# stevewongv/Sparse2Dense

Measured on AMD Instinct MI355X. Metric: LiDAR frames/sec (fwd+bwd), 150k-pt 0.1m-voxel synthetic Waymo scene, higher is better.
Workload: dtype bf16 (sparse stack: bf16 storage; dense neck/head: bf16 NHWC activations; fp32 accumulate, statistics, master weights, optimizer)

## Files before the change

include/s2d.h:

```cpp
#ifndef S2D_H_
#define S2D_H_

#include <stddef.h>
#include <stdint.h>

#ifdef __cplusplus
extern "C" {
#endif

typedef void *s2d_stream_t;

#define S2D_OK 0
#define S2D_ERR_INVALID_ARG (-1)
#define S2D_ERR_UNSUPPORTED (-2)
#define S2D_ERR_CAPACITY (-3)
#define S2D_ERR_WORKSPACE (-4)
#define S2D_ERR_COMM (-5)

int s2d_version(void);
int s2d_last_error(char *buf, size_t buf_len);
int s2d_build_info(char *buf, size_t buf_len);

size_t s2d_voxelize_batch_workspace_bytes(int frames, const int64_t *point_offsets, int max_points, int max_voxels);
int s2d_voxelize_batch_run(const float *points, int frames, const int64_t *point_offsets, int ndim,
// ... 179 lines not shown
                             s2d_stream_t stream);
int s2d_bnrow_apply_ld_bf16(const void *x, const float *scale, const float *shift, const void *residual, int relu, int64_t n, int c, void *y,
                            int y_ld, s2d_stream_t stream);
int s2d_bnrow_bwd_reduce_ld_bf16(const void *dy, int dy_ld, const void *x, const void *y, const float *scale, const float *shift, int relu,
                                 int64_t n, int c, float *sums, float *sums_copy, void *ws, size_t ws_bytes, s2d_stream_t stream);
int s2d_bnrow_bwd_reduce_finalize_ld_bf16(const void *dy, int dy_ld, const void *x, const void *y, const float *scale, const float *shift,
                                          int relu, int64_t n, int c, const float *gamma, const float *mean, const float *invstd,
                                          float *dgamma, float *dbeta, float *a, float *b, float *d, void *ws, size_t ws_bytes,
                                          s2d_stream_t stream);
int s2d_bnrow_bwd_apply_ld_bf16(const void *dy, int dy_ld, const void *x, const void *y, const float *scale, const float *shift, int relu,
                                const float *a, const float *b, const float *d, int64_t n, int c, void *dx, void *dres,
                                s2d_stream_t stream);

int s2d_spconv_s16_supported(int cin, int cout);
size_t s2d_spconv_s16_packed_elems(int kvol, int cin, int cout);
int s2d_spconv_s16_pack_weights(const float *weight, int kvol, int cin, int cout, int transpose,
                                int flip, int64_t n_out, void *packed, s2d_stream_t stream);
int s2d_spconv_s16_pack_weights_pair(const float *weight, int kvol, int cin, int cout, int flip_dgrad, int64_t n_out_fwd, int64_t n_out_dgrad,
                                     void *packed_fwd, void *packed_dgrad, s2d_stream_t stream);
int s2d_spconv_s16_wgrad(const void *in_feat, int64_t n_in, const void *dout, const int32_t *nbr,
                         int64_t n_out, int kvol, int cin, int cout, float *dweight, void *ws,
                         size_t ws_bytes, s2d_stream_t stream);
int s2d_spconv_s16_fwd(const void *in_feat, int64_t n_in, const void *packed_weight,
                       const float *bias, const int32_t *nbr, int64_t n_out, int kvol, int cin,
                       int cout, const void *zero_page, void *out_feat, s2d_stream_t stream);
int64_t s2d_spconv_s16_stats_tiles(int64_t n_out, int kvol, int cin, int cout);
int s2d_spconv_s16_fwd_stats(const void *in_feat, int64_t n_in, const void *packed_weight, const float *bias, const int32_t *nbr,
                             int64_t n_out, int kvol, int cin, int cout, const void *zero_page, void *out_feat, float *stats_partial,
                             s2d_stream_t stream);

int s2d_spconv_s16_set_sorted_rows(int on);
size_t s2d_rulebook_sort_workspace_bytes(int64_t n);
int64_t s2d_rulebook_sort_chunk_rows(int64_t n);
int s2d_rulebook_sort_by_mask(const int32_t *nbr, int kvol, int64_t n, int32_t *perm, uint32_t *pmask, int32_t *nbr_perm, void *ws,
                              size_t ws_bytes, s2d_stream_t stream);
int s2d_spconv_s16_sorted_supported(int kvol, int cin, int cout);
int s2d_spconv_s16_fwd_sorted(const void *in_feat, int64_t n_in, const void *packed_weight, const float *bias, const int32_t *nbr_perm,
                              const int32_t *perm, const uint32_t *pmask, int64_t n_out, int kvol, int cin, int cout, void *out_feat,
                              float *stats_partial, s2d_stream_t stream);

int s2d_conv2d3x3_wgrad_supported(int cin, int cout);
size_t s2d_conv2d3x3_wgrad_workspace_bytes(int n_img, int h, int w, int cin, int cout, int pad);
int s2d_conv2d3x3_wgrad_nhwc_bf16(const void *x, const void *dy, const void *zero_page, int n_img,
                                  int h, int w, int cin, int cout, int pad, float *dweight, float *dbias , void *ws,
                                  size_t ws_bytes, s2d_stream_t stream);

int s2d_conv2d1x1_pack_weights_bf16(const float *weight, int cin, int cout, int transpose, void *packed, s2d_stream_t stream);
int s2d_conv2d3x3_pack_weights_pair_bf16(const float *weight, int cin, int cout, int weight_nhwc, void *packed_fwd, void *packed_dgrad,
                                         s2d_stream_t stream);
int s2d_conv2d1x1_pack_weights_pair_bf16(const float *weight, int cin, int cout, void *packed_fwd, void *packed_dgrad, s2d_stream_t stream);
int64_t s2d_conv2d1x1_stats_tiles(int n_img, int h, int w, int cin, int cout);
int s2d_conv2d1x1_nhwc_bf16(const void *x, const void *packed_weight, const float *bias, const void *zero_page, int n_img,
                            int h, int w, int cin, int cout, void *y, float *stats_partial, s2d_stream_t stream);
size_t s2d_conv2d1x1_wgrad_workspace_bytes(int n_img, int h, int w, int cin, int cout);
int s2d_conv2d1x1_wgrad_nhwc_bf16(const void *x, const void *dy, const void *zero_page, int n_img, int h, int w, int cin,
                                  int cout, float *dweight, float *dbias , void *ws, size_t ws_bytes, s2d_stream_t stream);

int s2d_smallconv3x3_supported(int cin, int cout);
int s2d_smallconv3x3_fwd(const void *x, const float *weight, const float *bias, int n_img, int h, int w, int cin, int cout, float *y,
                         s2d_stream_t stream);
int s2d_smallconv3x3_dgrad(const float *dy, const float *weight, int n_img, int h, int w, int cin, int cout, void *dx,
                           s2d_stream_t stream);
size_t s2d_smallconv3x3_wgrad_workspace_bytes(int cin, int cout);
int s2d_smallconv3x3_wgrad(const void *x, const float *dy, int n_img, int h, int w, int cin, int cout, float *dweight, float *dbias,
                           void *ws, size_t ws_bytes, s2d_stream_t stream);

int s2d_conv2d2x2s2_pack_weights_bf16(const float *weight, int cin, int cout, int weight_nhwc, void *packed, s2d_stream_t stream);
int64_t s2d_conv2d2x2s2_stats_tiles(int n_img, int h, int w);
int s2d_conv2d2x2s2_nhwc_bf16(const void *x, const void *packed_weight, const float *bias, const void *zero_page, int n_img,
                              int h, int w, int cin, int cout, void *y, float *stats_partial, s2d_stream_t stream);

int s2d_convup_supported(int kc, int nc, int ks);
int s2d_convup_pack_weights_bf16(const float *weight, int kc, int nc, int ks, void *packed, s2d_stream_t stream);
int64_t s2d_convup_stats_tiles(int n_img, int h, int w, int kc, int nc, int ks);
int s2d_convup_nhwc_bf16(const void *x, const void *packed_weight, const float *bias, const void *zero_page, int n_img, int h, int w,
                         int kc, int nc, int ks, void *y, float *stats_partial, s2d_stream_t stream);
int s2d_conv2d4x4s2_pack_weights_bf16(const float *weight, int cin, int cout, void *packed, s2d_stream_t stream);
int s2d_conv2d4x4s2_nhwc_bf16(const void *x, const void *packed_weight, const void *zero_page, int n_img, int h, int w, int cin,
                              int cout, void *y, s2d_stream_t stream);
int s2d_conv2d_s2_wgrad_supported(int ca, int cb, int ks);
size_t s2d_conv2d_s2_wgrad_workspace_bytes(int n_img, int h, int w, int ca, int cb, int ks);
int s2d_conv2d_s2_wgrad_nhwc_bf16(const void *a, const void *b, const void *zero_page, int n_img, int h, int w, int ca, int cb, int ks,
                                  float *dweight, void *ws, size_t ws_bytes, s2d_stream_t stream);

int s2d_rows_wgrad_supported(int ci, int co);
size_t s2d_rows_wgrad_workspace_bytes(int64_t rows, int ci, int co);
int s2d_rows_wgrad_f32(const float *x, const float *dy, int64_t rows, int ci, int co, float *dweight, void *ws, size_t ws_bytes,
                       s2d_stream_t stream);

int s2d_dwconv7_supported(int channels);
int s2d_dwconv7_nhwc_bf16(const void *x, const float *weight, const float *bias, int n_img, int h, int w,
                          int c, int flip, void *y, s2d_stream_t stream);
size_t s2d_dwconv7_wgrad_workspace_bytes(int n_img, int h, int w, int c);
int s2d_dwconv7_wgrad_nhwc_bf16(const void *x, const void *dy, int n_img, int h, int w, int c,
                                float *dweight, float *dbias, void *ws, size_t ws_bytes,
                                s2d_stream_t stream);

int s2d_convt3d_mfma_supported(int cin, int cout);
size_t s2d_convt3d_mfma_packed_elems(int cin, int cout);
int s2d_convt3d_mfma_pack_weights(const float *weight, int cin, int cout, void *packed, s2d_stream_t stream);
int s2d_convt3d_mfma_fwd(const float *in, const void *packed, const float *bias, int batch, int cin, int cout,
                         int d, int h, int w, float *out, s2d_stream_t stream);
int64_t s2d_convt3d_mfma_stats_tiles(int batch, int cin, int d, int h, int w);
int s2d_convt3d_mfma_fwd_stats(const float *in, const void *packed, const float *bias, int batch, int cin, int cout,
                               int d, int h, int w, float *out, float *stats_partial, s2d_stream_t stream);
int s2d_convt3d_mfma_dgrad(const float *dout, const void *packed, int batch, int cin, int cout, int d, int h,
// ... 398 lines not shown
```

sparse2dense_amd/_lib.py:

```python
import ctypes
import os

_HERE = os.path.dirname(os.path.abspath(__file__))
LIB_PATH = os.path.join(_HERE, "lib", "libs2d_hip.so")

c_i32p = ctypes.c_void_p
c_f32p = ctypes.c_void_p
_I3 = ctypes.c_int32 * 3
_PFN_GEO = [ctypes.c_int64, ctypes.c_int, ctypes.c_int, ctypes.c_float, ctypes.c_float, ctypes.c_float, ctypes.c_float]
_F3 = ctypes.c_float * 3
_F6 = ctypes.c_float * 6


class CenterTask(ctypes.Structure):
    _fields_ = [(n, ctypes.c_void_p) for n in ("hm_logit", "reg", "height", "dim", "vel", "rot", "hm", "ind", "mask", "cat", "anno_box", "p",
                                               "d_logit", "d_reg", "d_height", "d_dim", "d_vel", "d_rot")] + [("classes", ctypes.c_int)]

class CenterPredictTask(ctypes.Structure):
    _fields_ = [("map", ctypes.c_void_p * 6), ("channel_stride", ctypes.c_int64 * 6), ("pixel_stride", ctypes.c_int64 * 6),
                ("classes", ctypes.c_int), ("label_base", ctypes.c_int)]


class AnchorPredictTask(ctypes.Structure):
    _fields_ = [(n, ctypes.c_void_p) for n in ("box_preds", "cls_preds", "dir_cls_preds", "anchors")] + \
# ... 94 lines not shown
                                              ctypes.c_int64, c_f32p, ctypes.c_void_p]),
    "s2d_comm_load_library": (ctypes.c_int, [ctypes.c_char_p]),
    "s2d_comm_available": (ctypes.c_int, []),
    "s2d_comm_unique_id": (ctypes.c_int, [ctypes.c_void_p]),
    "s2d_comm_init": (ctypes.c_int, [ctypes.c_void_p, ctypes.c_int, ctypes.c_int]),
    "s2d_comm_ranks": (ctypes.c_int, []),
    "s2d_comm_shutdown": (ctypes.c_int, []),
    "s2d_convt3d_mfma_supported": (ctypes.c_int, [ctypes.c_int, ctypes.c_int]),
    "s2d_convt3d_mfma_packed_elems": (ctypes.c_size_t, [ctypes.c_int, ctypes.c_int]),
    "s2d_convt3d_mfma_pack_weights": (ctypes.c_int, [c_f32p, ctypes.c_int, ctypes.c_int, ctypes.c_void_p, ctypes.c_void_p]),
    "s2d_convt3d_mfma_fwd": (ctypes.c_int, [c_f32p, ctypes.c_void_p, c_f32p] + [ctypes.c_int] * 6 + [c_f32p, ctypes.c_void_p]),
    "s2d_convt3d_mfma_stats_tiles": (ctypes.c_int64, [ctypes.c_int] * 5),
    "s2d_convt3d_mfma_fwd_stats": (ctypes.c_int, [c_f32p, ctypes.c_void_p, c_f32p] + [ctypes.c_int] * 6 + [c_f32p, c_f32p, ctypes.c_void_p]),
    "s2d_convt3d_mfma_fwd_stats_y16": (ctypes.c_int, [c_f32p, ctypes.c_void_p, c_f32p] + [ctypes.c_int] * 6 + [c_f32p, c_f32p, ctypes.c_void_p]),
    "s2d_convt3d_mfma_d16_supported": (ctypes.c_int, [ctypes.c_int] * 5),
    "s2d_convt3d_mfma_dgrad_d16": (ctypes.c_int, [ctypes.c_void_p, ctypes.c_void_p] + [ctypes.c_int] * 6 + [c_f32p, ctypes.c_void_p]),
    "s2d_convt3d_mfma_wgrad_d16": (ctypes.c_int, [c_f32p, ctypes.c_void_p] + [ctypes.c_int] * 6 + [c_f32p, ctypes.c_void_p, ctypes.c_size_t,
                                                                                                   ctypes.c_void_p]),
    "s2d_convt3d_mfma_norm_supported": (ctypes.c_int, [ctypes.c_int] * 5),
    "s2d_convt3d_mfma_fwd_stats_y16_norm": (ctypes.c_int, [c_f32p, c_f32p, ctypes.c_void_p, c_f32p] + [ctypes.c_int] * 6 + [ctypes.c_void_p, c_f32p,
                                                                                                                  ctypes.c_void_p]),
    "s2d_convt3d_mfma_wgrad_d16_norm": (ctypes.c_int, [c_f32p, c_f32p, ctypes.c_void_p] + [ctypes.c_int] * 6 + [c_f32p, ctypes.c_void_p, ctypes.c_size_t,
                                                                                                              ctypes.c_void_p]),
    "s2d_convt3d_mfma_dgrad": (ctypes.c_int, [c_f32p, ctypes.c_void_p] + [ctypes.c_int] * 6 + [c_f32p, ctypes.c_void_p]),
    "s2d_convt3d_mfma_wgrad_workspace_bytes": (ctypes.c_size_t, [ctypes.c_int] * 6),
    "s2d_convt3d_mfma_wgrad": (ctypes.c_int, [c_f32p, c_f32p] + [ctypes.c_int] * 6 + [c_f32p, ctypes.c_void_p, ctypes.c_size_t,
                                                                                     ctypes.c_void_p]),
    "s2d_pointwise_conv_wgrad_workspace_bytes": (ctypes.c_size_t, [ctypes.c_int, ctypes.c_int]),
    "s2d_pointwise_conv_wgrad_f32": (ctypes.c_int, [c_f32p, c_f32p, ctypes.c_int, ctypes.c_int, ctypes.c_int, ctypes.c_int64, c_f32p, c_f32p,
                                                    ctypes.c_void_p, ctypes.c_size_t, ctypes.c_void_p]),
    "s2d_pointwise_conv_wgrad_bf16_supported": (ctypes.c_int, [ctypes.c_int, ctypes.c_int, ctypes.c_int64]),
    "s2d_pointwise_conv_wgrad_norm_bf16": (ctypes.c_int, [c_f32p, c_f32p, c_f32p, ctypes.c_int, ctypes.c_int, ctypes.c_int, ctypes.c_int64, c_f32p,
                                                          c_f32p, ctypes.c_void_p, ctypes.c_size_t, ctypes.c_void_p]),
    "s2d_pointwise_conv_wgrad_norm_x16": (ctypes.c_int, [c_f32p, c_f32p, c_f32p, ctypes.c_int, ctypes.c_int, ctypes.c_int, ctypes.c_int64, c_f32p,
                                                          c_f32p, ctypes.c_void_p, ctypes.c_size_t, ctypes.c_void_p]),
    "s2d_pointwise_conv_wgrad_bf16": (ctypes.c_int, [c_f32p, c_f32p, ctypes.c_int, ctypes.c_int, ctypes.c_int, ctypes.c_int64, c_f32p, c_f32p,
                                                     ctypes.c_void_p, ctypes.c_size_t, ctypes.c_void_p]),
    "s2d_pcr_loss_workspace_bytes": (ctypes.c_size_t, []),
    "s2d_pcr_loss_fwd_f32": (ctypes.c_int, [c_f32p, c_f32p, c_i32p, c_f32p, ctypes.c_int64] + [ctypes.c_int] * 4 +
                             [c_f32p, ctypes.c_void_p, ctypes.c_size_t, ctypes.c_void_p]),
    "s2d_pcr_loss_bwd_f32": (ctypes.c_int, [c_f32p, c_f32p, c_i32p, c_f32p, ctypes.c_int64] + [ctypes.c_int] * 4 +
                             [c_f32p, c_f32p, c_f32p, c_f32p, c_f32p, ctypes.c_void_p]),
    "s2d_nhwc_bf16_to_nchw_f32": (ctypes.c_int, [ctypes.c_void_p, ctypes.c_int, ctypes.c_int, ctypes.c_int64, c_f32p, ctypes.c_void_p]),
    "s2d_nchw_f32_to_nhwc_bf16": (ctypes.c_int, [c_f32p, ctypes.c_int, ctypes.c_int, ctypes.c_int64, ctypes.c_void_p, ctypes.c_void_p]),
    "s2d_nhwc_bf16_to_nchw_f32_ld": (ctypes.c_int, [ctypes.c_void_p, ctypes.c_int, ctypes.c_int, ctypes.c_int, ctypes.c_int64, c_f32p, ctypes.c_void_p]),
    "s2d_nchw_f32_to_nhwc_bf16_ld": (ctypes.c_int, [c_f32p, ctypes.c_int, ctypes.c_int, ctypes.c_int, ctypes.c_int64, ctypes.c_void_p, ctypes.c_void_p]),
    "s2d_conv2d1x1_pack_weights_bf16": (ctypes.c_int, [c_f32p, ctypes.c_int, ctypes.c_int, ctypes.c_int, ctypes.c_void_p, ctypes.c_void_p]),
    "s2d_conv2d3x3_pack_weights_pair_bf16": (ctypes.c_int, [c_f32p, ctypes.c_int, ctypes.c_int, ctypes.c_int, ctypes.c_void_p, ctypes.c_void_p,
                                                            ctypes.c_void_p]),
    "s2d_conv2d1x1_pack_weights_pair_bf16": (ctypes.c_int, [c_f32p, ctypes.c_int, ctypes.c_int, ctypes.c_void_p, ctypes.c_void_p, ctypes.c_void_p]),
    "s2d_conv2d1x1_stats_tiles": (ctypes.c_int64, [ctypes.c_int] * 5),
    "s2d_conv2d1x1_nhwc_bf16": (ctypes.c_int, [ctypes.c_void_p, ctypes.c_void_p, c_f32p, ctypes.c_void_p] + [ctypes.c_int] * 5 +
                                [ctypes.c_void_p, c_f32p, ctypes.c_void_p]),
    "s2d_conv2d1x1_wgrad_workspace_bytes": (ctypes.c_size_t, [ctypes.c_int] * 5),
    "s2d_conv2d1x1_wgrad_nhwc_bf16": (ctypes.c_int, [ctypes.c_void_p, ctypes.c_void_p, ctypes.c_void_p] + [ctypes.c_int] * 5 +
                                      [c_f32p, c_f32p, ctypes.c_void_p, ctypes.c_size_t, ctypes.c_void_p]),
    "s2d_smallconv3x3_supported": (ctypes.c_int, [ctypes.c_int, ctypes.c_int]),
    "s2d_smallconv3x3_fwd": (ctypes.c_int, [ctypes.c_void_p, c_f32p, c_f32p] + [ctypes.c_int] * 5 + [c_f32p, ctypes.c_void_p]),
    "s2d_smallconv3x3_dgrad": (ctypes.c_int, [c_f32p, c_f32p] + [ctypes.c_int] * 5 + [ctypes.c_void_p, ctypes.c_void_p]),
    "s2d_smallconv3x3_wgrad_workspace_bytes": (ctypes.c_size_t, [ctypes.c_int, ctypes.c_int]),
    "s2d_smallconv3x3_wgrad": (ctypes.c_int, [ctypes.c_void_p, c_f32p] + [ctypes.c_int] * 5 +
                               [c_f32p, c_f32p, ctypes.c_void_p, ctypes.c_size_t, ctypes.c_void_p]),
    "s2d_conv2d2x2s2_pack_weights_bf16": (ctypes.c_int, [c_f32p, ctypes.c_int, ctypes.c_int, ctypes.c_int, ctypes.c_void_p, ctypes.c_void_p]),
    "s2d_conv2d2x2s2_stats_tiles": (ctypes.c_int64, [ctypes.c_int, ctypes.c_int, ctypes.c_int]),
    "s2d_conv2d2x2s2_nhwc_bf16": (ctypes.c_int, [ctypes.c_void_p, ctypes.c_void_p, c_f32p, ctypes.c_void_p] + [ctypes.c_int] * 5 +
                                  [ctypes.c_void_p, c_f32p, ctypes.c_void_p]),
    "s2d_convup_supported": (ctypes.c_int, [ctypes.c_int] * 3),
    "s2d_convup_pack_weights_bf16": (ctypes.c_int, [c_f32p, ctypes.c_int, ctypes.c_int, ctypes.c_int, ctypes.c_void_p, ctypes.c_void_p]),
    "s2d_convup_stats_tiles": (ctypes.c_int64, [ctypes.c_int] * 6),
    "s2d_convup_nhwc_bf16": (ctypes.c_int, [ctypes.c_void_p, ctypes.c_void_p, c_f32p, ctypes.c_void_p] + [ctypes.c_int] * 6 +
                             [ctypes.c_void_p, c_f32p, ctypes.c_void_p]),
    "s2d_conv2d4x4s2_pack_weights_bf16": (ctypes.c_int, [c_f32p, ctypes.c_int, ctypes.c_int, ctypes.c_void_p, ctypes.c_void_p]),
    "s2d_conv2d4x4s2_nhwc_bf16": (ctypes.c_int, [ctypes.c_void_p, ctypes.c_void_p, ctypes.c_void_p] + [ctypes.c_int] * 5 +
                                  [ctypes.c_void_p, ctypes.c_void_p]),
    "s2d_conv2d_s2_wgrad_supported": (ctypes.c_int, [ctypes.c_int] * 3),
    "s2d_conv2d_s2_wgrad_workspace_bytes": (ctypes.c_size_t, [ctypes.c_int] * 6),
    "s2d_conv2d_s2_wgrad_nhwc_bf16": (ctypes.c_int, [ctypes.c_void_p, ctypes.c_void_p, ctypes.c_void_p] + [ctypes.c_int] * 6 +
                                      [c_f32p, ctypes.c_void_p, ctypes.c_size_t, ctypes.c_void_p]),
    "s2d_rows_wgrad_supported": (ctypes.c_int, [ctypes.c_int, ctypes.c_int]),
    "s2d_rows_wgrad_workspace_bytes": (ctypes.c_size_t, [ctypes.c_int64, ctypes.c_int, ctypes.c_int]),
    "s2d_rows_wgrad_f32": (ctypes.c_int, [c_f32p, c_f32p, ctypes.c_int64, ctypes.c_int, ctypes.c_int, c_f32p, ctypes.c_void_p, ctypes.c_size_t,
                                          ctypes.c_void_p]),
    "s2d_lnwide_workspace_bytes": (ctypes.c_size_t, [ctypes.c_int]),
    "s2d_lnwide_fwd_bf16": (ctypes.c_int, [ctypes.c_void_p, c_f32p, c_f32p, ctypes.c_int, ctypes.c_int64, ctypes.c_float, ctypes.c_void_p, c_f32p,
                                           ctypes.c_void_p, ctypes.c_size_t, ctypes.c_void_p]),
    "s2d_lnwide_bwd_bf16": (ctypes.c_int, [ctypes.c_void_p, ctypes.c_void_p, c_f32p, c_f32p, ctypes.c_int, ctypes.c_int64, ctypes.c_void_p, c_f32p,
                                           c_f32p, ctypes.c_void_p, ctypes.c_size_t, ctypes.c_void_p]),
    "s2d_focal_workspace_bytes": (ctypes.c_size_t, []),
    "s2d_focal_fwd": (ctypes.c_int, [c_f32p, c_f32p, ctypes.c_void_p, ctypes.c_void_p, ctypes.c_void_p, ctypes.c_int, ctypes.c_int, ctypes.c_int64,
                                     ctypes.c_int, c_f32p, ctypes.c_void_p, ctypes.c_size_t, ctypes.c_void_p]),
    "s2d_focal_bwd": (ctypes.c_int, [c_f32p, c_f32p, ctypes.c_void_p, ctypes.c_void_p, ctypes.c_void_p, ctypes.c_int, ctypes.c_int, ctypes.c_int64,
                                     ctypes.c_int, c_f32p, c_f32p, c_f32p, ctypes.c_void_p]),
    "s2d_regloss_fwd": (ctypes.c_int, [c_f32p, ctypes.c_void_p, ctypes.c_void_p, c_f32p, ctypes.c_int, ctypes.c_int, ctypes.c_int64, ctypes.c_int,
                                       c_f32p, ctypes.c_void_p]),
    "s2d_regloss_bwd": (ctypes.c_int, [c_f32p, ctypes.c_void_p, ctypes.c_void_p, c_f32p, ctypes.c_int, ctypes.c_int, ctypes.c_int64, ctypes.c_int,
                                       c_f32p, c_f32p, c_f32p, ctypes.c_void_p]),
    "s2d_center_tasks_loss_workspace_bytes": (ctypes.c_size_t, []),
    "s2d_center_tasks_loss_fwd": (ctypes.c_int, [ctypes.c_void_p, ctypes.c_int, ctypes.c_int, ctypes.c_int64, ctypes.c_int, c_f32p, ctypes.c_float,
                                                 c_f32p, c_f32p, c_f32p, ctypes.c_void_p, ctypes.c_size_t, ctypes.c_void_p]),
    "s2d_center_tasks_loss_bwd": (ctypes.c_int, [ctypes.c_void_p, ctypes.c_int, ctypes.c_int, ctypes.c_int64, ctypes.c_int, c_f32p, ctypes.c_float,
                                                 c_f32p, c_f32p, c_f32p, ctypes.c_void_p, ctypes.c_size_t, ctypes.c_void_p]),
    "s2d_masked_mse_workspace_bytes": (ctypes.c_size_t, []),
    "s2d_masked_mse_fwd": (ctypes.c_int, [ctypes.c_void_p, ctypes.c_int, ctypes.c_void_p, ctypes.c_int, ctypes.c_int64, ctypes.c_float, ctypes.c_float,
                                          c_f32p, ctypes.c_void_p, ctypes.c_size_t, ctypes.c_void_p]),
    "s2d_masked_mse_bwd": (ctypes.c_int, [ctypes.c_void_p, ctypes.c_int, ctypes.c_void_p, ctypes.c_int, ctypes.c_int64, c_f32p, c_f32p,
                                          ctypes.c_void_p, ctypes.c_void_p]),
# ... 328 lines not shown
```

sparse2dense_amd/build.py:

```python
import glob
import os
import subprocess
import sys

HERE = os.path.dirname(os.path.abspath(__file__))
CSRC = os.path.join(HERE, "csrc")
LIBDIR = os.path.join(HERE, "lib")
LIB = os.path.join(LIBDIR, "libs2d_hip.so")
HIPCC = os.environ.get("HIPCC", "/opt/rocm/bin/hipcc")
FLAGS = ["--offload-arch=gfx950", "-O3", "-std=c++17", "-fPIC", "-Wall", "-Wno-unused-function",
         "-fno-fast-math", "-ffp-contract=off"]


EXTRA = {"deform_conv.hip": ["-fno-slp-vectorize"], "center_predict.hip": ["-fno-slp-vectorize"], "roi_head.hip": ["-fno-slp-vectorize"],
         "anchor_predict.hip": ["-fno-slp-vectorize"], "roi_mlp.hip": ["-fno-slp-vectorize"], "pillar_distill.hip": ["-fno-slp-vectorize"],
         "prep.hip": ["-fno-slp-vectorize"], "tracking.hip": ["-fno-slp-vectorize"]}
if os.environ.get("S2D_BUILD_LOSSES_SLP") != "1":
    EXTRA["losses.hip"] = ["-fno-slp-vectorize"]


def _stale(target, deps):
    if not os.path.exists(target):
        return True
    t = os.path.getmtime(target)
    return any(os.path.getmtime(d) > t for d in deps)


def build(force=False, verbose=True):
    os.makedirs(LIBDIR, exist_ok=True)
    objdir = os.path.join(LIBDIR, "obj")
    os.makedirs(objdir, exist_ok=True)
    srcs = sorted(glob.glob(os.path.join(CSRC, "*.hip")))
    hdrs = sorted(glob.glob(os.path.join(CSRC, "*.h"))) + [os.path.join(os.path.dirname(HERE), "include", "s2d.h")]
    objs = []
    procs = []
    for s in srcs:
        o = os.path.join(objdir, os.path.basename(s)[:-4] + ".o")
        objs.append(o)
        flags = FLAGS + EXTRA.get(os.path.basename(s), [])
        stamp = o[:-2] + ".flags"
        built_with = open(stamp).read() if os.path.exists(stamp) else " ".join(FLAGS)
        if force or _stale(o, [s] + hdrs) or built_with != " ".join(flags):
            for stale in (o, stamp):
                if os.path.exists(stale):
                    os.remove(stale)
            cmd = [HIPCC] + flags + ["-c", s, "-o", o]
            if verbose:
                print(" ".join(cmd), file=sys.stderr, flush=True)
            procs.append((s, subprocess.Popen(cmd), stamp, " ".join(flags)))
    failed = []
    for s, p, stamp, flag_line in procs:
        if p.wait() != 0:
            failed.append(s)
            continue
        with open(stamp, "w") as f:
            f.write(flag_line)
    if failed:
        raise RuntimeError(f"hipcc failed on {failed}")
    if force or procs or _stale(LIB, objs):
        cmd = [HIPCC, "--offload-arch=gfx950", "-shared", "-fPIC", "-o", LIB] + objs
        if verbose:
            print(" ".join(cmd), file=sys.stderr, flush=True)
        subprocess.check_call(cmd)
    return LIB


if __name__ == "__main__":
# ... 2 lines not shown
```

sparse2dense_amd/csrc/conv2d_nhwc.hip:

```cpp
#include "s2d_common.h"
#include <cstdlib>

namespace s2d {

typedef float f32x4c __attribute__((ext_vector_type(4)));
typedef __bf16 bf16x8c __attribute__((ext_vector_type(8)));
typedef __bf16 bf16x4c __attribute__((ext_vector_type(4)));

__device__ __forceinline__ void conv2d_pack_element(const float *__restrict__ w, int cin, int cout, int bn, int transpose_flip, int w_nhwc, int taps,
                                                    int64_t i, __bf16 *__restrict__ out) {
    const int64_t total = (int64_t)taps * cin * cout;
    if (i >= total) return;
    const int ntile = bn / 16, per_wave = bn / 32;
    int64_t r = i;
    const int e = r % 8; r /= 8;
    const int c = r % 16; r /= 16;
    const int q = r % 4; r /= 4;
    const int nt = r % ntile; r /= ntile;
    const int h = r % 2; r /= 2;
    const int blk = r % (cout / bn); r /= (cout / bn);
    const int chunk = r % (cin / 64); r /= (cin / 64);
    const int tap = (int)r;
    const int ci = chunk * 64 + h * 32 + 8 * q + e;
    const int co = blk * bn + (nt / per_wave) * (bn / 2) + c * per_wave + (nt % per_wave);
// ... 1106 lines not shown
    if (!s2d_conv2d3x3_supported(cin, cout)) {
        set_error("conv2d4x4s2_pack: unsupported channels %d -> %d", cin, cout);
        return S2D_ERR_UNSUPPORTED;
    }
    const int64_t total = (int64_t)16 * cin * cout;
    hipLaunchKernelGGL(conv2d_pack_kernel, dim3((unsigned)ceil_div(total, 256)), dim3(256), 0, (hipStream_t)stream, weight, cin, cout,
                       conv_bn(cout), 0, 0, 16, (__bf16 *)packed);
    S2D_LAUNCH_CHECK();
    return S2D_OK;
}

extern "C" int s2d_conv2d4x4s2_nhwc_bf16(const void *x, const void *packed_weight, const void *zero_page, int n_img, int h, int w, int cin,
                                         int cout, void *y, s2d_stream_t stream) {
    S2D_CHECK_ARG(x && packed_weight && zero_page && y && n_img > 0 && h >= 2 && w >= 2 && h % 2 == 0 && w % 2 == 0,
                  "conv2d4x4s2: bad argument");
    if (!s2d_conv2d3x3_supported(cin, cout)) {
        set_error("conv2d4x4s2: unsupported channels %d -> %d", cin, cout);
        return S2D_ERR_UNSUPPORTED;
    }
    const int64_t m = (int64_t)n_img * (h / 2) * (w / 2);
    hipStream_t st = (hipStream_t)stream;
    if (conv_bn(cout) == 64) {
        hipLaunchKernelGGL((conv3x3_k32_nhwc_bf16_kernel<64, 4, 4, false>), dim3(xcd_grid(ceil_div(m, 128)), cout / 64), dim3(256),
                           3 * (size_t)(128 * 64 + 64 * 64), st, (const __bf16 *)x, (const __bf16 *)packed_weight, (const float *)nullptr,
                           (const __bf16 *)zero_page, n_img, h, w, cin, cout, 1, 2, (__bf16 *)y, (float *)nullptr, BnBwd{});
        S2D_LAUNCH_CHECK();
        return S2D_OK;
    }
    const int rows = conv_k32_rows(m, cout / 128);
#define S2D_CONV4(MI_)                                                                                                             \
    hipLaunchKernelGGL((conv3x3_k32_nhwc_bf16_kernel<128, MI_, 4, false>), dim3(xcd_grid(ceil_div(m, 32 * MI_)), cout / 128),       \
                       dim3(256), 3 * (size_t)(32 * MI_ * 64 + 64 * 128), st, (const __bf16 *)x, (const __bf16 *)packed_weight,    \
                       (const float *)nullptr, (const __bf16 *)zero_page, n_img, h, w, cin, cout, 1, 2, (__bf16 *)y, (float *)nullptr, BnBwd{})
    if (rows == 128) S2D_CONV4(4); else if (rows == 96) S2D_CONV4(3); else S2D_CONV4(2);
#undef S2D_CONV4
    S2D_LAUNCH_CHECK();
    return S2D_OK;
}


extern "C" int s2d_conv2d1x1_pack_weights_bf16(const float *weight, int cin, int cout, int transpose, void *packed, s2d_stream_t stream) {
    S2D_CHECK_ARG(weight && packed, "conv2d1x1_pack: null argument");
    if (!s2d_conv2d3x3_supported(cin, cout)) {
        set_error("conv2d1x1_pack: unsupported channels %d -> %d", cin, cout);
        return S2D_ERR_UNSUPPORTED;
    }
    const int64_t total = (int64_t)cin * cout;
    hipLaunchKernelGGL(conv2d_pack_kernel, dim3((unsigned)ceil_div(total, 256)), dim3(256), 0, (hipStream_t)stream, weight, cin, cout,
                       conv_bn(cout), transpose, 0, 1, (__bf16 *)packed);
    S2D_LAUNCH_CHECK();
    return S2D_OK;
}

static bool conv1x1_use_k32(int cin) {
    static const bool k64 = [] { const char *e = getenv("S2D_CONV1X1"); return e && e[0] == 'k' && e[1] == '6'; }();
    return !k64 && cin >= 128;
}
static int conv1x1_rows(int64_t m, int cin, int cout) {
    return conv1x1_use_k32(cin) && conv_bn(cout) == 128 ? conv_k32_rows(m, cout / 128) : 128;
}

extern "C" int64_t s2d_conv2d1x1_stats_tiles(int n_img, int h, int w, int cin, int cout) {
    const int64_t m = (int64_t)n_img * h * w;
    return ceil_div(m, conv1x1_rows(m, cin, cout));
}

static int conv1x1_run(const void *x, const void *packed_weight, const float *bias, const void *zero_page, int n_img, int h, int w, int cin,
                       int cout, void *y, float *stats_partial, const BnBwd bb, s2d_stream_t stream) {
    S2D_CHECK_ARG(x && packed_weight && zero_page && y && n_img > 0 && h > 0 && w > 0, "conv2d1x1: bad argument");
    if (!s2d_conv2d3x3_supported(cin, cout)) {
        set_error("conv2d1x1: unsupported channels %d -> %d", cin, cout);
        return S2D_ERR_UNSUPPORTED;
    }
    const int64_t m = (int64_t)n_img * h * w;
    const int bn = conv_bn(cout);
    const dim3 grid(xcd_grid(ceil_div(m, 128)), cout / bn), blk(256);
    const size_t lds = (size_t)2 * (128 * 64 * 2 + 64 * bn * 2);
    hipStream_t st = (hipStream_t)stream;
    if (bb.z && !conv1x1_use_k32(cin)) {
        set_error("conv2d1x1: the batch-norm backward epilogue needs the 32-deep kernel (%d -> %d)", cin, cout);
        return S2D_ERR_UNSUPPORTED;
    }
    if (conv1x1_use_k32(cin)) {
#define S2D_CONV1_K32(BN_, MI_)                                                                                                    \
    hipLaunchKernelGGL((conv3x3_k32_nhwc_bf16_kernel<BN_, MI_, 1, false>), dim3(xcd_grid(ceil_div(m, 32 * MI_)), cout / bn), blk,   \
                       3 * (size_t)(32 * MI_ * 64 + 64 * BN_), st, (const __bf16 *)x, (const __bf16 *)packed_weight, bias,         \
                       (const __bf16 *)zero_page, n_img, h, w, cin, cout, 0, 1, (__bf16 *)y, stats_partial, bb)
        if (bn == 128) {
            const int rows = conv1x1_rows(m, cin, cout);
            if (rows == 128) S2D_CONV1_K32(128, 4); else if (rows == 96) S2D_CONV1_K32(128, 3); else S2D_CONV1_K32(128, 2);
        } else {
            S2D_CONV1_K32(64, 4);
        }
#undef S2D_CONV1_K32
        S2D_LAUNCH_CHECK();
        return S2D_OK;
    }
#define S2D_CONV1_LAUNCH(BN_)                                                                                             \
    do {                                                                                                                  \
        auto kern = conv3x3_nhwc_bf16_kernel<BN_, 2, 1>;                                                                  \
        static bool attr_set = false;                                                                                     \
        if (!attr_set) {                                                                                                  \
            S2D_HIP(hipFuncSetAttribute((const void *)kern, hipFuncAttributeMaxDynamicSharedMemorySize, (int)lds));       \
            attr_set = true;                                                                                              \
        }                                                                                                                 \
        hipLaunchKernelGGL(kern, grid, blk, lds, st, (const __bf16 *)x, (const __bf16 *)packed_weight, bias,              \
                           (const __bf16 *)zero_page, n_img, h, w, cin, cout, 0, 1, (__bf16 *)y, stats_partial);          \
    } while (0)
    if (bn == 128) S2D_CONV1_LAUNCH(128); else S2D_CONV1_LAUNCH(64);
#undef S2D_CONV1_LAUNCH
    S2D_LAUNCH_CHECK();
    return S2D_OK;
}

extern "C" int s2d_conv2d1x1_nhwc_bf16(const void *x, const void *packed_weight, const float *bias, const void *zero_page, int n_img, int h,
                                       int w, int cin, int cout, void *y, float *stats_partial, s2d_stream_t stream) {
    return conv1x1_run(x, packed_weight, bias, zero_page, n_img, h, w, cin, cout, y, stats_partial, BnBwd{}, stream);
}

extern "C" int s2d_conv2d1x1_bnbwd_supported(int cin, int cout) { return s2d_conv2d3x3_supported(cin, cout) && conv1x1_use_k32(cin); }

extern "C" int s2d_conv2d1x1_nhwc_bf16_bnbwd(const void *x, const void *packed_weight, const void *zero_page, int n_img, int h, int w, int cin,
                                             int cout, void *y, const void *bn_z, const float *bn_scale, const float *bn_shift, int bn_act,
                                             float *bn_partial, s2d_stream_t stream) {
    S2D_CHECK_ARG(bn_z && bn_scale && bn_shift && bn_partial && bn_act >= 0 && bn_act <= 2, "conv2d1x1_bnbwd: bad argument");
    BnBwd bb;
    bb.z = (const __bf16 *)bn_z; bb.scale = bn_scale; bb.shift = bn_shift; bb.act = bn_act;
    return conv1x1_run(x, packed_weight, nullptr, zero_page, n_img, h, w, cin, cout, y, bn_partial, bb, stream);
}


extern "C" int s2d_conv2d2x2s2_pack_weights_bf16(const float *weight, int cin, int cout, int weight_nhwc, void *packed, s2d_stream_t stream) {
    S2D_CHECK_ARG(weight && packed, "conv2d2x2s2_pack: null argument");
    if (!s2d_conv2d3x3_supported(cin, cout)) {
// ... 41 lines not shown
```

sparse2dense_amd/dense2d.py:

```python
import ctypes

import torch

from . import collective as _collective
from torch import nn
import torch.nn.functional as F

from . import _lib
from ._lib import check

ENABLED = True

_zero_pages = {}


def _zero_page(device):
    z = _zero_pages.get(device)
    if z is None:
        z = torch.zeros(64, dtype=torch.uint8, device=device)
        _zero_pages[device] = z
    return z


def _ptr(t):
# ... 350 lines not shown
            if self.emit_bn_stats and self.training and torch.is_grad_enabled():
                y, partial = _Conv3x3Fn.apply(x, self.weight, self.bias, pad, self.stride[0], True, src)
                y._s2d_bn_partial = partial
                return y
            return _Conv3x3Fn.apply(x, self.weight, self.bias, pad, self.stride[0], False, src)
        if self.absorbed_pad:
            x = torch.nn.functional.pad(x, (self.absorbed_pad,) * 4)
        return super().forward(x)


def _pack_weights_1x1(weight, transpose, with_dgrad=False):
    if with_dgrad and not transpose and not cached_pack_has(weight, ("conv1x1", False)) and not cached_pack_has(weight, ("conv1x1", True)):
        lib = _lib.load()
        cout, cin = weight.shape[0], weight.shape[1]
        if lib.s2d_conv2d3x3_supported(cin, cout) and lib.s2d_conv2d3x3_supported(cout, cin):
            w = weight.detach().float().reshape(cout, cin).contiguous()
            pf = torch.empty(cin * cout, dtype=torch.bfloat16, device=weight.device)
            pd = torch.empty(cin * cout, dtype=torch.bfloat16, device=weight.device)
            launch = lambda: check(lib.s2d_conv2d1x1_pack_weights_pair_bf16(_ptr(w), cin, cout, _ptr(pf), _ptr(pd), _stream()),
                                   "s2d_conv2d1x1_pack_weights_pair_bf16")
            launch()
            cached_pack_put(weight, ("conv1x1", False), pf)
            cached_pack_put(weight, ("conv1x1", True), pd)
            register_repack(weight, [("conv1x1", False), ("conv1x1", True)], w, launch, conv2d=(w, cin, cout, 1, 0, 0, pf, pd))

    def build():
        lib = _lib.load()
        cout, cin = weight.shape[0], weight.shape[1]
        w = weight.detach().float().reshape(cout, cin).contiguous()
        packed = torch.empty(cin * cout, dtype=torch.bfloat16, device=weight.device)
        pc_in, pc_out = (cout, cin) if transpose else (cin, cout)
        launch = lambda: check(lib.s2d_conv2d1x1_pack_weights_bf16(_ptr(w), pc_in, pc_out, int(transpose), _ptr(packed), _stream()),
                               "s2d_conv2d1x1_pack_weights_bf16")
        launch()
        register_repack(weight, [("conv1x1", bool(transpose))], w, launch, conv2d=(w, pc_in, pc_out, 1, 0, int(transpose), packed, None))
        return packed
    return cached_pack(weight, ("conv1x1", bool(transpose)), build)


def conv1x1_nhwc(x, packed, bias, cin, cout, bn_stats=False, bn_bwd=None):
    lib = _lib.load()
    assert x.dtype == torch.bfloat16 and x.is_contiguous(memory_format=torch.channels_last) and x.shape[1] == cin
    n, _, h, w = x.shape
    y = torch.empty((n, cout, h, w), dtype=torch.bfloat16, device=x.device, memory_format=torch.channels_last)
    partial = (torch.empty((lib.s2d_conv2d1x1_stats_tiles(n, h, w, cin, cout), 2, cout), dtype=torch.float32, device=x.device)
               if (bn_stats or bn_bwd is not None) else None)
    from . import hip_ops as H
    rec = None
    if H.PROFILE is not None:
        tiles = lib.s2d_conv2d1x1_stats_tiles(n, h, w, cin, cout)
        rows = next(bm for bm in (128, 96, 64) if -(-n * h * w // bm) == tiles)
        bn = 128 if cout % 128 == 0 else 64
        k32 = cin >= 128 and _os.environ.get("S2D_CONV1X1", "")[:2] != "k6"
        rec = dict(kernel="conv1x1_nhwc_bf16", tag="dense1x1", cin=cin, cout=cout, n_out=n * h * w, kvol=1, pairs=None, dense=True,
                   in_pixels=n * h * w, pad=0, stride=1, tile_rows=rows,
                   kname=(f"conv3x3_k32_nhwc_bf16_kernel<{bn}, {rows // 32}, 1, false>" if k32 else f"conv3x3_nhwc_bf16_kernel<{bn}, 2, 1>"),
                   start=torch.cuda.Event(enable_timing=True), end=torch.cuda.Event(enable_timing=True))
        rec["start"].record()
    if bn_bwd is not None:
        z, fin, act = bn_bwd[0], bn_bwd[1], bn_bwd[2]
        assert bias is None and not bn_stats and z.shape == y.shape and z.dtype == torch.bfloat16 \
            and z.is_contiguous(memory_format=torch.channels_last) and fin.shape == (4, cout)
        fp = fin.data_ptr()
        check(lib.s2d_conv2d1x1_nhwc_bf16_bnbwd(_ptr(x), _ptr(packed), _ptr(_zero_page(x.device)), n, h, w, cin, cout, _ptr(y), _ptr(z),
                                                fp + 8 * cout, fp + 12 * cout, int(act), _ptr(partial), _stream()),
              "s2d_conv2d1x1_nhwc_bf16_bnbwd")
    else:
        check(lib.s2d_conv2d1x1_nhwc_bf16(_ptr(x), _ptr(packed), _ptr(bias), _ptr(_zero_page(x.device)), n, h, w, cin, cout, _ptr(y),
                                          _ptr(partial), _stream()), "s2d_conv2d1x1_nhwc_bf16")
    if rec is not None:
        rec["end"].record()
        H.PROFILE.append(rec)
    return (y, partial) if (bn_stats or bn_bwd is not None) else y


def _pack_matrix_1x1(owner, tag, make, transpose=False):
    def build():
        lib = _lib.load()
        m = make().detach().float().contiguous()
        out_c, in_c = m.shape
        packed = torch.empty(out_c * in_c, dtype=torch.bfloat16, device=m.device)
        pc_in, pc_out = (out_c, in_c) if transpose else (in_c, out_c)
        check(lib.s2d_conv2d1x1_pack_weights_bf16(_ptr(m), pc_in, pc_out, int(transpose), _ptr(packed), _stream()),
              "s2d_conv2d1x1_pack_weights_bf16")
        return packed
    return cached_pack(owner, tag, build)


def _space_depth_hip(t):
    return (ENABLED and t.is_cuda and t.dtype == torch.bfloat16 and t.dim() == 4 and t.shape[1] % 8 == 0 and t.numel() > 0
            and t.is_contiguous(memory_format=torch.channels_last) and not (t.requires_grad and torch.is_grad_enabled()))


def _space_to_depth(t):
    n, c, hh, ww = t.shape
    if _space_depth_hip(t) and hh % 2 == 0 and ww % 2 == 0:
        y = torch.empty((n, 4 * c, hh // 2, ww // 2), dtype=torch.bfloat16, device=t.device, memory_format=torch.channels_last)
        check(_lib.load().s2d_space_depth2_nhwc_bf16(_ptr(t), n, hh // 2, ww // 2, c, 1, _ptr(y), _stream()), "s2d_space_depth2_nhwc_bf16")
        return y
    v = t.permute(0, 2, 3, 1).reshape(n, hh // 2, 2, ww // 2, 2, c).permute(0, 1, 3, 2, 4, 5).reshape(n, hh // 2, ww // 2, 4 * c)
    return v.permute(0, 3, 1, 2)


def _depth_to_space(t, c):
    n, _, h, w = t.shape
    if _space_depth_hip(t) and t.shape[1] == 4 * c and c % 8 == 0:
        y = torch.empty((n, c, 2 * h, 2 * w), dtype=torch.bfloat16, device=t.device, memory_format=torch.channels_last)
        check(_lib.load().s2d_space_depth2_nhwc_bf16(_ptr(t), n, h, w, c, 0, _ptr(y), _stream()), "s2d_space_depth2_nhwc_bf16")
        return y
# ... 771 lines not shown
```

Measured before the change: 222.8.

## Add persistent weight-resident 1x1 conv forward kernel for large NHWC pointwise layers

Adds a new persistent pointwise-conv forward kernel. Each workgroup loads its output-column block's packed weights (up to two 128-channel blocks) into LDS once, then loops over a contiguous range of row tiles with MFMA 16x16x32 bf16, register double-buffered B fragments and prefetched A rows. The grid is sized to the CU count. The path is taken for large pixel counts with cout=256 (cin 128, or cin 256 without stats), replacing the generic k32 conv kernel. This is meant to cut repeated weight fetches and per-tile launch overhead, at the cost of up to 160KB of LDS per block, which gives low occupancy.

```diff
diff --git a/include/s2d.h b/include/s2d.h
--- a/include/s2d.h
+++ b/include/s2d.h
@@ -255,6 +255,8 @@
 int64_t s2d_conv2d1x1_stats_tiles(int n_img, int h, int w, int cin, int cout);
 int s2d_conv2d1x1_nhwc_bf16(const void *x, const void *packed_weight, const float *bias, const void *zero_page, int n_img,
                             int h, int w, int cin, int cout, void *y, float *stats_partial, s2d_stream_t stream);
+int s2d_conv2d1x1_set_route(int route);
+int s2d_conv2d1x1_plan(int n_img, int h, int w, int cin, int cout, int with_stats);
 size_t s2d_conv2d1x1_wgrad_workspace_bytes(int n_img, int h, int w, int cin, int cout);
 int s2d_conv2d1x1_wgrad_nhwc_bf16(const void *x, const void *dy, const void *zero_page, int n_img, int h, int w, int cin,
                                   int cout, float *dweight, float *dbias , void *ws, size_t ws_bytes, s2d_stream_t stream);
diff --git a/sparse2dense_amd/_lib.py b/sparse2dense_amd/_lib.py
--- a/sparse2dense_amd/_lib.py
+++ b/sparse2dense_amd/_lib.py
@@ -170,6 +170,8 @@
     "s2d_conv2d1x1_stats_tiles": (ctypes.c_int64, [ctypes.c_int] * 5),
     "s2d_conv2d1x1_nhwc_bf16": (ctypes.c_int, [ctypes.c_void_p, ctypes.c_void_p, c_f32p, ctypes.c_void_p] + [ctypes.c_int] * 5 +
                                 [ctypes.c_void_p, c_f32p, ctypes.c_void_p]),
+    "s2d_conv2d1x1_set_route": (ctypes.c_int, [ctypes.c_int]),
+    "s2d_conv2d1x1_plan": (ctypes.c_int, [ctypes.c_int] * 6),
     "s2d_conv2d1x1_wgrad_workspace_bytes": (ctypes.c_size_t, [ctypes.c_int] * 5),
     "s2d_conv2d1x1_wgrad_nhwc_bf16": (ctypes.c_int, [ctypes.c_void_p, ctypes.c_void_p, ctypes.c_void_p] + [ctypes.c_int] * 5 +
                                       [c_f32p, c_f32p, ctypes.c_void_p, ctypes.c_size_t, ctypes.c_void_p]),
diff --git a/sparse2dense_amd/build.py b/sparse2dense_amd/build.py
--- a/sparse2dense_amd/build.py
+++ b/sparse2dense_amd/build.py
@@ -12,7 +12,8 @@
          "-fno-fast-math", "-ffp-contract=off"]
 
 
-EXTRA = {"deform_conv.hip": ["-fno-slp-vectorize"], "center_predict.hip": ["-fno-slp-vectorize"], "roi_head.hip": ["-fno-slp-vectorize"],
+EXTRA = {"pointwise_nhwc.hip": ["-fno-slp-vectorize"],
+         "deform_conv.hip": ["-fno-slp-vectorize"], "center_predict.hip": ["-fno-slp-vectorize"], "roi_head.hip": ["-fno-slp-vectorize"],
          "anchor_predict.hip": ["-fno-slp-vectorize"], "roi_mlp.hip": ["-fno-slp-vectorize"], "pillar_distill.hip": ["-fno-slp-vectorize"],
          "prep.hip": ["-fno-slp-vectorize"], "tracking.hip": ["-fno-slp-vectorize"]}
 if os.environ.get("S2D_BUILD_LOSSES_SLP") != "1":
diff --git a/sparse2dense_amd/csrc/conv2d_nhwc.hip b/sparse2dense_amd/csrc/conv2d_nhwc.hip
--- a/sparse2dense_amd/csrc/conv2d_nhwc.hip
+++ b/sparse2dense_amd/csrc/conv2d_nhwc.hip
@@ -1182,6 +1182,11 @@
     return S2D_OK;
 }
 
+namespace s2d {
+int pointwise_fwd_plan(int64_t m, int cin, int cout, int rows, bool with_stats, bool bnbwd);
+int pointwise_fwd_launch(const void *x, const void *wpack, const float *bias, int64_t m, int cin, int cout, int rows, void *y, float *stats,
+                         hipStream_t st);
+}
 static bool conv1x1_use_k32(int cin) {
     static const bool k64 = [] { const char *e = getenv("S2D_CONV1X1"); return e && e[0] == 'k' && e[1] == '6'; }();
     return !k64 && cin >= 128;
@@ -1193,6 +1198,12 @@
 extern "C" int64_t s2d_conv2d1x1_stats_tiles(int n_img, int h, int w, int cin, int cout) {
     const int64_t m = (int64_t)n_img * h * w;
     return ceil_div(m, conv1x1_rows(m, cin, cout));
+}
+
+extern "C" int s2d_conv2d1x1_plan(int n_img, int h, int w, int cin, int cout, int with_stats) {
+    if (n_img <= 0 || h <= 0 || w <= 0 || !s2d_conv2d3x3_supported(cin, cout) || !conv1x1_use_k32(cin)) return 0;
+    const int64_t m = (int64_t)n_img * h * w;
+    return pointwise_fwd_plan(m, cin, cout, conv1x1_rows(m, cin, cout), with_stats != 0, false);
 }
 
 static int conv1x1_run(const void *x, const void *packed_weight, const float *bias, const void *zero_page, int n_img, int h, int w, int cin,
@@ -1210,6 +1221,11 @@
     if (bb.z && !conv1x1_use_k32(cin)) {
         set_error("conv2d1x1: the batch-norm backward epilogue needs the 32-deep kernel (%d -> %d)", cin, cout);
         return S2D_ERR_UNSUPPORTED;
+    }
+    if (conv1x1_use_k32(cin)) {
+        const int rows = conv1x1_rows(m, cin, cout);
+        if (pointwise_fwd_plan(m, cin, cout, rows, stats_partial != nullptr, bb.z != nullptr))
+            return pointwise_fwd_launch(x, packed_weight, bias, m, cin, cout, rows, y, stats_partial, st);
     }
     if (conv1x1_use_k32(cin)) {
 #define S2D_CONV1_K32(BN_, MI_)                                                                                                    \
diff --git a/sparse2dense_amd/csrc/pointwise_nhwc.hip b/sparse2dense_amd/csrc/pointwise_nhwc.hip
--- /dev/null
+++ b/sparse2dense_amd/csrc/pointwise_nhwc.hip
@@ -0,0 +1,243 @@
+#include "s2d_common.h"
+#include <cstdlib>
+
+namespace s2d {
+
+typedef float f32x4p __attribute__((ext_vector_type(4)));
+typedef __bf16 bf16x8p __attribute__((ext_vector_type(8)));
+typedef __bf16 bf16x4p __attribute__((ext_vector_type(4)));
+
+template <int BN, int MI>
+__device__ __forceinline__ void pw_epilogue(f32x4p (&acc)[MI][BN / 32], const float *bias_blk, __bf16 *__restrict__ y, int64_t m0,
+                                            int64_t m_total, int cout, int cb, int wm, int wn, int r, int q, float *red,
+                                            float *__restrict__ stats_partial, int tile) {
+    constexpr int NT = BN / 32;
+    const int co_base = cb * BN + wn * (BN / 2);
+    float bv[NT], s1[NT], s2[NT];
+#pragma unroll
+    for (int j = 0; j < NT; ++j) {
+        bv[j] = bias_blk[wn * (BN / 2) + r * NT + j];
+        s1[j] = 0.f;
+        s2[j] = 0.f;
+    }
+#pragma unroll
+    for (int i = 0; i < MI; ++i)
+#pragma unroll
+        for (int reg = 0; reg < 4; ++reg) {
+            const int64_t m = m0 + 16 * MI * wm + 16 * i + 4 * q + reg;
+            if (m < m_total) {
+                __bf16 v[NT];
+#pragma unroll
+                for (int j = 0; j < NT; ++j) {
+                    v[j] = (__bf16)(acc[i][j][reg] + bv[j]);
+                    const float f = (float)v[j];
+                    s1[j] += f;
+                    s2[j] += f * f;
+                }
+                __bf16 *dst = y + m * cout + co_base + r * NT;
+                if (NT == 4) {
+                    bf16x4p o;
+                    o[0] = v[0]; o[1] = v[1 % NT]; o[2] = v[2 % NT]; o[3] = v[3 % NT];
+                    *reinterpret_cast<bf16x4p *>(dst) = o;
+                } else {
+                    dst[0] = v[0];
+                    dst[1] = v[1 % NT];
+                }
+            }
+        }
+    if (stats_partial) {
+#pragma unroll
+        for (int j = 0; j < NT; ++j) {
+            s1[j] += __shfl_xor(s1[j], 16, 64); s1[j] += __shfl_xor(s1[j], 32, 64);
+            s2[j] += __shfl_xor(s2[j], 16, 64); s2[j] += __shfl_xor(s2[j], 32, 64);
+        }
+        __builtin_amdgcn_s_waitcnt(0xc07f);
+        __builtin_amdgcn_s_barrier();
+        if (q == 0) {
+#pragma unroll
+            for (int j = 0; j < NT; ++j) {
+                red[(wm * 2 + 0) * BN + wn * (BN / 2) + r * NT + j] = s1[j];
+                red[(wm * 2 + 1) * BN + wn * (BN / 2) + r * NT + j] = s2[j];
+            }
+        }
+        __builtin_amdgcn_s_waitcnt(0xc07f);
+        __builtin_amdgcn_s_barrier();
+        for (int e = threadIdx.x; e < 2 * BN; e += 256) {
+            const int which = e / BN, col = e - which * BN;
+            stats_partial[((int64_t)tile * 2 + which) * cout + cb * BN + col] = red[which * BN + col] + red[(2 + which) * BN + col];
+        }
+    }
+}
+
+template <int CIN, int MI, int NCW>
+__device__ __forceinline__ void pw_resident_tiles(const __bf16 *__restrict__ x, int64_t m_total, int cout, __bf16 *__restrict__ y,
+                                                  float *__restrict__ stats_partial, int t0, int t1, int cb0, float *red,
+                                                  const float *bias_lds, const char *bres) {
+    constexpr int BN = 128, NT = 4;
+    constexpr int KS = CIN / 32;
+    constexpr int BM = 32 * MI;
+    constexpr int B_HALF = 64 * BN;
+    const int lane = threadIdx.x & 63;
+    const int wid = __builtin_amdgcn_readfirstlane(threadIdx.x >> 6);
+    const int wm = wid >> 1, wn = wid & 1;
+    const int r = lane & 15, q = lane >> 4;
+    bf16x8p a[KS][MI];
+    const __bf16 *a_ptr[MI];
+    auto set_rows = [&](int tile) {
+#pragma unroll
+        for (int i = 0; i < MI; ++i) {
+            int64_t m = (int64_t)tile * BM + 16 * MI * wm + 16 * i + r;
+            m = m < m_total ? m : m_total - 1;
+            a_ptr[i] = x + m * CIN + 8 * q;
+        }
+    };
+    auto load_step = [&](int s) {
+#pragma unroll
+        for (int i = 0; i < MI; ++i) a[s][i] = *reinterpret_cast<const bf16x8p *>(a_ptr[i] + s * 32);
+    };
+    const char *b_rd = bres + (wn * NT * 64 + lane) * 16;
+    auto read_b = [&](int s, bf16x8p (&fb)[NCW][NT]) {
+#pragma unroll
+        for (int c = 0; c < NCW; ++c)
+#pragma unroll
+            for (int j = 0; j < NT; ++j) fb[c][j] = *reinterpret_cast<const bf16x8p *>(b_rd + (size_t)(c * KS + s) * B_HALF + j * 1024);
+    };
+    set_rows(t0);
+#pragma unroll
+    for (int s = 0; s < KS; ++s) load_step(s);
+    for (int tile = t0; tile < t1; ++tile) {
+        set_rows(tile + 1 < t1 ? tile + 1 : tile);
+        f32x4p acc[NCW][MI][NT];
+#pragma unroll
+        for (int c = 0; c < NCW; ++c)
+#pragma unroll
+            for (int i = 0; i < MI; ++i)
+#pragma unroll
+                for (int j = 0; j < NT; ++j) acc[c][i][j] = f32x4p{0.f, 0.f, 0.f, 0.f};
+        bf16x8p fb[2][NCW][NT];
+        read_b(0, fb[0]);
+#pragma unroll
+        for (int s = 0; s < KS; ++s) {
+            if (s + 1 < KS) read_b(s + 1, fb[(s + 1) & 1]);
+#pragma unroll
+            for (int c = 0; c < NCW; ++c)
+#pragma unroll
+                for (int i = 0; i < MI; ++i)
+#pragma unroll
+                    for (int j = 0; j < NT; ++j)
+                        acc[c][i][j] = __builtin_amdgcn_mfma_f32_16x16x32_bf16(a[s][i], fb[s & 1][c][j], acc[c][i][j], 0, 0, 0);
+            load_step(s);
+            __builtin_amdgcn_sched_barrier(0);
+        }
+#pragma unroll
+        for (int c = 0; c < NCW; ++c)
+            pw_epilogue<BN, MI>(acc[c], bias_lds + c * BN, y, (int64_t)tile * BM, m_total, cout, cb0 + c, wm, wn, r, q, red, stats_partial, tile);
+    }
+}
+
+template <int CIN, int MI>
+__global__ __launch_bounds__(256) void pointwise_resident_kernel(const __bf16 *__restrict__ x, const __bf16 *__restrict__ wpack,
+                                                                 const float *__restrict__ bias, int64_t m_total, int cout,
+                                                                 __bf16 *__restrict__ y, float *__restrict__ stats_partial, int tiles,
+                                                                 int wgs_per_block) {
+    constexpr int BN = 128, CBW = 2;
+    constexpr int KS = CIN / 32;
+    constexpr int B_HALF = 64 * BN;
+    extern __shared__ __attribute__((aligned(16))) char smem[];
+    float *red = reinterpret_cast<float *>(smem);
+    float *bias_lds = red + 4 * BN;
+    char *bres = smem + (4 + CBW) * BN * 4;
+
+    const int lane = threadIdx.x & 63;
+    const int wid = __builtin_amdgcn_readfirstlane(threadIdx.x >> 6);
+    const int ncb = cout / BN;
+    const int cb0 = (int)(blockIdx.x / wgs_per_block) / CBW * CBW;
+    const int ncw = ncb - cb0 < CBW ? ncb - cb0 : CBW;
+    const int gsize = ncw * wgs_per_block, gidx = (int)blockIdx.x - cb0 * wgs_per_block;
+    const int t0 = (int)((int64_t)gidx * tiles / gsize), t1 = (int)((int64_t)(gidx + 1) * tiles / gsize);
+    if (t1 <= t0) return;
+
+    for (int c = threadIdx.x; c < ncw * BN; c += 256) bias_lds[c] = bias ? bias[cb0 * BN + c] : 0.f;
+    {
+        const char *wbytes = reinterpret_cast<const char *>(wpack);
+        const int total = ncw * KS * (B_HALF / 1024);
+        for (int idx = wid; idx < total; idx += 4) {
+            const int unit = idx % (B_HALF / 1024), cs = idx / (B_HALF / 1024), s = cs % KS, c = cs / KS;
+            const char *src = wbytes + ((int64_t)((s >> 1) * ncb + cb0 + c) * 2 + (s & 1)) * B_HALF + unit * 1024 + lane * 16;
+            __builtin_amdgcn_global_load_lds((const __attribute__((address_space(1))) void *)src,
+                                             (__attribute__((address_space(3))) void *)(bres + (size_t)idx * 1024), 16, 0, 0);
+        }
+    }
+    __syncthreads();
+
+    if (ncw == 2) pw_resident_tiles<CIN, MI, 2>(x, m_total, cout, y, stats_partial, t0, t1, cb0, red, bias_lds, bres);
+    else pw_resident_tiles<CIN, MI, 1>(x, m_total, cout, y, stats_partial, t0, t1, cb0, red, bias_lds, bres);
+}
+
+static int g_route = -1;
+int conv1x1_route() {
+    if (g_route < 0) {
+        const char *e = getenv("S2D_CONV1X1");
+        g_route = (e && (e[0] == '1' || e[0] == '2') && !e[1]) ? e[0] - '0' : 0;
+    }
+    return g_route;
+}
+
+static int pw_cus() {
+    static int n = 0;
+    if (!n) {
+        int dev = 0;
+        if (hipGetDevice(&dev) != hipSuccess || hipDeviceGetAttribute(&n, hipDeviceAttributeMultiprocessorCount, dev) != hipSuccess || n <= 0) n = 256;
+    }
+    return n;
+}
+
+constexpr size_t PW_LDS = 160 * 1024;
+
+int pointwise_fwd_plan(int64_t m, int cin, int cout, int rows, bool with_stats, bool bnbwd) {
+    const int route = conv1x1_route();
+    if (route == 1 || bnbwd) return 0;
+    if ((cin != 128 && cin != 256) || cout < 128 || cout % 128 || (rows != 128 && rows != 96 && rows != 64)) return 0;
+    if (route == 2) return 1;
+    return m >= 100000 && cout == 256 && (cin == 128 || !with_stats) ? 1 : 0;
+}
+
+template <int CIN, int MI>
+static int pw_launch_resident(const void *x, const void *wpack, const float *bias, int64_t m, int cout, void *y, float *stats, hipStream_t st) {
+    const int ncb = cout / 128;
+    const size_t lds = (4 + 2) * 128 * 4 + (size_t)(ncb < 2 ? ncb : 2) * CIN * 128 * 2;
+    auto kern = pointwise_resident_kernel<CIN, MI>;
+    static bool attr_set = false;
+    if (!attr_set) {
+        S2D_HIP(hipFuncSetAttribute((const void *)kern, hipFuncAttributeMaxDynamicSharedMemorySize, (int)PW_LDS));
+        attr_set = true;
+    }
+    const int64_t tiles = ceil_div(m, 32 * MI);
+    int wpb = pw_cus() / ncb;
+    if (wpb < 1) wpb = 1;
+    if (wpb > tiles) wpb = (int)tiles;
+    hipLaunchKernelGGL(kern, dim3((unsigned)(ncb * wpb)), dim3(256), lds, st, (const __bf16 *)x, (const __bf16 *)wpack, bias, m, cout,
+                       (__bf16 *)y, stats, (int)tiles, wpb);
+    S2D_LAUNCH_CHECK();
+    return S2D_OK;
+}
+
+int pointwise_fwd_launch(const void *x, const void *wpack, const float *bias, int64_t m, int cin, int cout, int rows, void *y, float *stats,
+                         hipStream_t st) {
+    if (cin == 256) {
+        if (rows == 128) return pw_launch_resident<256, 4>(x, wpack, bias, m, cout, y, stats, st);
+        if (rows == 96) return pw_launch_resident<256, 3>(x, wpack, bias, m, cout, y, stats, st);
+        return pw_launch_resident<256, 2>(x, wpack, bias, m, cout, y, stats, st);
+    }
+    if (rows == 128) return pw_launch_resident<128, 4>(x, wpack, bias, m, cout, y, stats, st);
+    if (rows == 96) return pw_launch_resident<128, 3>(x, wpack, bias, m, cout, y, stats, st);
+    return pw_launch_resident<128, 2>(x, wpack, bias, m, cout, y, stats, st);
+}
+
+}
+
+extern "C" int s2d_conv2d1x1_set_route(int route) {
+    S2D_CHECK_ARG(route >= 0 && route <= 2, "conv2d1x1_set_route: route must be 0, 1 or 2");
+    s2d::g_route = route;
+    return S2D_OK;
+}
diff --git a/sparse2dense_amd/dense2d.py b/sparse2dense_amd/dense2d.py
--- a/sparse2dense_amd/dense2d.py
+++ b/sparse2dense_amd/dense2d.py
@@ -426,9 +426,11 @@
         rows = next(bm for bm in (128, 96, 64) if -(-n * h * w // bm) == tiles)
         bn = 128 if cout % 128 == 0 else 64
         k32 = cin >= 128 and _os.environ.get("S2D_CONV1X1", "")[:2] != "k6"
+        plan = 0 if bn_bwd is not None else lib.s2d_conv2d1x1_plan(n, h, w, cin, cout, int(partial is not None))
         rec = dict(kernel="conv1x1_nhwc_bf16", tag="dense1x1", cin=cin, cout=cout, n_out=n * h * w, kvol=1, pairs=None, dense=True,
                    in_pixels=n * h * w, pad=0, stride=1, tile_rows=rows,
-                   kname=(f"conv3x3_k32_nhwc_bf16_kernel<{bn}, {rows // 32}, 1, false>" if k32 else f"conv3x3_nhwc_bf16_kernel<{bn}, 2, 1>"),
+                   kname=(f"pointwise_resident_kernel<{cin}, {rows // 32}>" if plan else
+                          f"conv3x3_k32_nhwc_bf16_kernel<{bn}, {rows // 32}, 1, false>" if k32 else f"conv3x3_nhwc_bf16_kernel<{bn}, 2, 1>"),
                    start=torch.cuda.Event(enable_timing=True), end=torch.cuda.Event(enable_timing=True))
         rec["start"].record()
     if bn_bwd is not None:
```

Result: no change. 223.3 (median of 2 runs) (+0.2%).
